# afanasyev-ilya/VectorGraphLibrary

Hardware: AMD Instinct MI355X
Metric: TEPS (edges/s) BFS + SSSP on RMAT-24; value = direction-optimising BFS, sssp_value_teps = direction-optimising Bellman-Ford (higher is better)
Workload: dtype int32; 1 GPU; BFS direction-optimising on RMAT scale-24 (edge factor 32), 1xMI355X; vertices=16777216, edges=536870912, seed=1, parallelism=edge-cut x1, exchange_transport=none, vertex_numbering=degree-sorted (total)

## Files before the change

### profiles/microbench/bfs_launches.py

```python
#!/usr/bin/env python3
import csv
import glob
import sys

files = sorted(glob.glob(sys.argv[1] + "/**/*kernel_trace.csv", recursive=True))
rows = []
for f in files:
    with open(f) as fh:
        for r in csv.DictReader(fh):
            rows.append((int(r["Start_Timestamp"]), int(r["End_Timestamp"]), r["Kernel_Name"].split("(")[0]))
rows.sort()
short = {"vgl_k_bu_probe": "probe", "vgl_k_bu_heavy": "heavy", "vgl_k_bm_advance": "adv", "vgl_k_td_expand": "td"}
inits = [i for i, r in enumerate(rows) if "bfs_init" in r[2]]
n = int(sys.argv[2]) if len(sys.argv) > 2 else 3
spans = [(a, b) for a, b in zip(inits[:-1], inits[1:]) if any("bu_probe" in r[2] for r in rows[a:b])]
for a, b in spans[-n:]:
    t0 = rows[a][0]
    parts, prev_end, busy = [], None, 0
    for s, e, name in rows[a:b]:
        label = next((v for k, v in short.items() if k in name), name.replace('void ', '').replace('vgl_k_', '')[:14])
        gap = "" if prev_end is None else f"(+{(s - prev_end) / 1e3:.1f})"
        parts.append(f"{label} {(e - s) / 1e3:.1f}{gap}")
        busy += e - s
        prev_end = e
    span = rows[b - 1][1] - t0
    print("traversal: " + "  ".join(parts) + f"   | span {span / 1e3:.1f} us, kernels {busy / 1e3:.1f} us, idle {(span - busy) / 1e3:.1f} us")
```

### vectorgraphlibrary_amd/csrc/bfs.hip

```cpp
#include "vgl_hip_internal.h"
#include <chrono>
#include "vgl_gnf.h"
#include "vgl_blocked.h"

#ifndef VGL_BU_HEAVY_LANES
#define VGL_BU_HEAVY_LANES 16
#endif

__global__ __launch_bounds__(VGL_BLOCK) void vgl_k_bfs_init(int32_t V, int32_t source, int32_t *levels)
{
    for (int32_t v = blockIdx.x * VGL_BLOCK + threadIdx.x; v < V; v += gridDim.x * VGL_BLOCK)
        levels[v] = (v == source) ? 1 : -1;
}

__global__ __launch_bounds__(VGL_BLOCK) void vgl_k_bfs_init_all(int32_t V, int32_t source, int32_t *levels, int64_t words, uint64_t *visited,
                                                                uint64_t *front, uint64_t *next, uint32_t *tickets, unsigned long long *list_count)
{
    if (blockIdx.x == 0 && threadIdx.x == 0) *list_count = 0ULL;
    for (int32_t v = blockIdx.x * VGL_BLOCK + threadIdx.x; v < V; v += gridDim.x * VGL_BLOCK)
        levels[v] = (v == source) ? 1 : -1;
    for (int64_t w = (int64_t)blockIdx.x * VGL_BLOCK + threadIdx.x; w < words; w += (int64_t)gridDim.x * VGL_BLOCK) {
        const uint64_t bit = (w == (source >> 6)) ? (1ULL << (source & 63)) : 0ULL;
        visited[w] = bit; front[w] = bit; next[w] = 0;
    }
// ... 556 lines not shown
            for (int u = 0; u < U; u++) {
                const unsigned long long bit = dst[u] >= 0 ? 1ULL << (dst[u] & 63) : 0ULL;
                old[u] = (word[u] & bit) || dst[u] < 0 ? ~0ULL : atomicOr((unsigned long long *)&visited[dst[u] >> 6], bit);
            }
#pragma unroll
            for (int u = 0; u < U; u++) {
                if (dst[u] < 0) continue;
                const unsigned long long bit = 1ULL << (dst[u] & 63);
                if (old[u] & bit) continue;
                levels[dst[u]] = level + 1;
                atomicOr((unsigned long long *)&next[dst[u] >> 6], bit);
                const int pos = atomicAdd(&s_cnt, 1);
                if (pos < VGL_SMALL_F) s_list[cur ^ 1][pos] = dst[u];
                else found_deg += rowptr[dst[u] + 1] - rowptr[dst[u]];
            }
        }
        __syncthreads();
        const int32_t Fn = s_cnt;
        edges += M; run++; last_f = F;
        if (run > 1) later_front += F;
        F = Fn;
        if (Fn > VGL_SMALL_F) {
            {
                static_assert(VGL_SMALL_F == 2 * NT, "two listed vertices per thread");
                const int32_t v0 = s_list[cur ^ 1][tid], v1 = s_list[cur ^ 1][tid + NT];
                const int64_t a0 = rowptr[v0], a1 = rowptr[v0 + 1], c0 = rowptr[v1], c1 = rowptr[v1 + 1];
                found_deg += (a1 - a0) + (c1 - c0);
            }
            found_deg = vgl_wave_incl_add(found_deg);
            if (lane == 63) s_deg[wave] = found_deg;
            __syncthreads();
#pragma unroll
            for (int w = 0; w < NW; w++) next_m += s_deg[w];
            hinted = 1;
            break;
        }
        if (Fn == 0) break;
        cur ^= 1; level++;
    }
    if (tid == 0) {
        counters[C_FRONT] = F; counters[C_TMP0] = run; counters[C_EDGES] = edges; counters[C_TMP1] = later_front; counters[C_JUMP] = last_f;
        counters[C_NEIGH] = first_m; counters[C_BU_FOUND] = n_list; counters[C_CHANGED] = bm_edges;
        if (hinted) { counters[C_NEXT_F] = F; counters[C_NEXT_M] = next_m; }
        host[C_HINT] = hinted;
        host[C_FRONT] = F; host[C_TMP0] = run; host[C_EDGES] = edges; host[C_TMP1] = later_front; host[C_JUMP] = last_f; host[C_NEIGH] = first_m;
        host[C_BU_FOUND] = n_list; host[C_CHANGED] = bm_edges; host[C_HEAVY] = handed; host[C_BU_EDGES] = exit_m;
        __threadfence_system();
        host[C_NSLOTS] = seq;
        __threadfence_system();
    }
}

constexpr int VGL_BU_BLOCKS = 2048;

typedef int vgl_int4_u __attribute__((ext_vector_type(4), aligned(4)));

typedef unsigned vgl_uint3_u __attribute__((ext_vector_type(3), aligned(4)));
template <bool PACKED>
__device__ __forceinline__ void vgl_load_head(const int4 *in_head, int64_t rec, int32_t u[4])
{
    if constexpr (PACKED) {
        const vgl_uint3_u w = *reinterpret_cast<const vgl_uint3_u *>(reinterpret_cast<const uint32_t *>(in_head) + 3 * rec);
        const uint32_t f[4] = {w.x & 0xFFFFFFu, (w.x >> 24) | ((w.y & 0xFFFFu) << 8), (w.y >> 16) | ((w.z & 0xFFu) << 16), w.z >> 8};
#pragma unroll
        for (int q = 0; q < 4; q++) u[q] = f[q] == 0xFFFFFFu ? -1 : (int32_t)f[q];
    } else {
        const int4 h = in_head[rec];
        u[0] = h.x; u[1] = h.y; u[2] = h.z; u[3] = h.w;
    }
}
template <bool INLINE_HEAVY, bool PACKED>
__device__ __forceinline__ void vgl_bu_probe_body(int32_t nrows, int32_t row_base, int32_t chunk, const int64_t *in_rowptr,
                                                  const int32_t *in_adj, const uint64_t *visited, const uint64_t *in_nz,
                                                  const uint64_t *front, uint64_t *next, int32_t *levels, int32_t next_level,
                                                  int32_t *heavy, int64_t *partials, uint32_t *ticket, const int4 *in_head,
                                                  const uint64_t *in_long, const int32_t *nz_rank, int32_t nz_rows, int64_t *counters,
                                                  volatile int64_t *host, int64_t seq)
{
    static_assert(INLINE_HEAVY, "the deferred rows are scanned in the same launch");
    __shared__ int64_t s64[VGL_WAVES];
    __shared__ int s_nheavy;
    if (threadIdx.x == 0) s_nheavy = 0;
    __syncthreads();
    auto in_front = [&](int32_t u) -> uint32_t { return (uint32_t)((front[u >> 6] >> (u & 63)) & 1ULL); };
    int64_t found_cnt = 0, probes = 0;
    const int64_t groups = ((int64_t)nrows + 63) >> 6;
    const int64_t word0 = (int64_t)row_base >> 6;
    constexpr int64_t NW = (int64_t)VGL_BU_BLOCKS * VGL_WAVES;
    int32_t *my_heavy = heavy + (int64_t)blockIdx.x * chunk;
    const int lane = vgl_lane();
    for (int64_t g0 = (int64_t)blockIdx.x * VGL_WAVES + vgl_wave(); g0 < groups; g0 += NW * 64) {
        const int64_t mine = g0 + (int64_t)lane * NW;
        uint64_t cw = 0, nzw = 0;
        int32_t nzr = 0;
        if (mine < groups) {
            nzw = in_nz[word0 + mine];
            cw = ~visited[word0 + mine] & nzw;
            if (cw == 0ULL) next[word0 + mine] = 0ULL;
            else nzr = nz_rank[mine];
        }
        unsigned long long todo = __ballot(cw != 0ULL);
        while (todo) {
            const int j = __ffsll((long long)todo) - 1;
            todo &= todo - 1;
            const uint64_t cand_word = __shfl(cw, j);
            const int32_t rec = __shfl(nzr, j) + (int32_t)__popcll(__shfl(nzw, j) & ((1ULL << lane) - 1ULL));
            const int64_t grp = g0 + (int64_t)j * NW;
            const int32_t r = (int32_t)(grp << 6) + lane;
            const int32_t v = row_base + r;
            bool found = false, defer = false;
            if (r < nrows && ((cand_word >> lane) & 1ULL)) {
                int32_t u0[4];
                vgl_load_head<PACKED>(in_head, rec, u0);
                uint32_t hit = 0;
                int n = 0;
#pragma unroll
                for (int q = 0; q < 4; q++) if (u0[q] >= 0) n = q + 1;
                if (u0[0] >= 0) hit = in_front(u0[0]);
                if (hit == 0) {
#pragma unroll
                    for (int q = 1; q < 4; q++)
                        if (u0[q] >= 0) hit |= in_front(u0[q]) << q;
                }
                bool longer = false;
                if (hit == 0 && n == 4) {
                    int32_t u1[4];
                    vgl_load_head<PACKED>(in_head, (int64_t)nz_rows + rec, u1);
#pragma unroll
                    for (int q = 0; q < 4; q++)
                        if (u1[q] >= 0) { n = 5 + q; hit |= in_front(u1[q]) << (4 + q); }
                    longer = (in_long[v >> 6] >> (v & 63)) & 1ULL;
                }
                found = hit != 0;
                probes += found ? __ffs(hit) : n;
                defer = !found && longer;
                if (found) levels[v] = next_level;
            }
            const unsigned long long fm = __ballot(found);
            if (lane == 0) next[word0 + grp] = fm;
            found_cnt += found;
            const unsigned long long dm = __ballot(defer);
            if (dm) {
                int base = 0;
                if (lane == 0) base = atomicAdd(&s_nheavy, (int)__popcll(dm));
                base = __shfl(base, 0);
                if (defer) my_heavy[base + __popcll(dm & ((1ULL << lane) - 1ULL))] = r;
            }
        }
    }
    __syncthreads();
    const int nh = s_nheavy;
    constexpr int G = VGL_BU_HEAVY_LANES, NG = 64 / G;
    const int quarter = lane / G, ql = lane % G;
    for (int h0 = vgl_wave() * NG; h0 < nh; h0 += VGL_WAVES * NG) {
        const int h = h0 + quarter;
        bool done = h >= nh, hit_any = false;
        int32_t r = 0;
        int64_t p = 0, e = 0;
        if (!done) { r = my_heavy[h]; p = in_rowptr[r]; e = in_rowptr[r + 1]; }
        while (!__all(done)) {
            const int64_t q = p + ql;
            bool hit = false;
            if (!done && q < e) { const int32_t u = in_adj[q]; hit = (front[u >> 6] >> (u & 63)) & 1ULL; }
            const unsigned long long hm = __ballot(hit);
            const unsigned qm = (unsigned)(hm >> (quarter * G)) & (G >= 32 ? 0xFFFFFFFFu : ((1u << (G & 31)) - 1u));
            if (!done) {
                if (qm) { hit_any = true; done = true; if (ql == 0) probes += __ffs(qm); }
                else { if (ql == 0) probes += min((int64_t)G, e - p); p += G; if (p >= e) done = true; }
            }
        }
        if (hit_any && ql == 0) {
            const int32_t v = row_base + r;
            levels[v] = next_level;
            atomicOr((unsigned long long *)&next[v >> 6], 1ULL << (v & 63));
            found_cnt++;
        }
    }
    found_cnt = vgl_block_reduce_add(found_cnt, s64);
    probes = vgl_block_reduce_add(probes, s64);
    uint32_t dep = 0;
    if (threadIdx.x == 0) dep = vgl_put_agent(partials + blockIdx.x * 4 + 0, found_cnt) ^ vgl_put_agent(partials + blockIdx.x * 4 + 1, probes);
    if (!vgl_last_block(ticket, dep)) return;
    int64_t f = 0, pr = 0;
    for (int b = threadIdx.x; b < (int)gridDim.x; b += VGL_BLOCK) { f += vgl_load_agent(partials + b * 4 + 0); pr += vgl_load_agent(partials + b * 4 + 1); }
    f = vgl_block_reduce_add(f, s64);
    pr = vgl_block_reduce_add(pr, s64);
    if (threadIdx.x == 0) {
        if (host) vgl_publish2(counters, host, seq, C_BU_FOUND, f, C_BU_EDGES, pr);
        else { counters[C_BU_FOUND] = f; counters[C_BU_EDGES] = pr; }
    }
}
#define VGL_BU_PROBE_PARAMS                                                                                                                             \
    int32_t nrows, int32_t row_base, int32_t chunk, const int64_t *in_rowptr, const int32_t *in_adj, const uint64_t *visited, const uint64_t *in_nz,  \
        const uint64_t *front, uint64_t *next, int32_t *levels, int32_t next_level, int32_t *heavy, int64_t *partials, uint32_t *ticket,               \
        const int4 *in_head, const uint64_t *in_long, const int32_t *nz_rank, int32_t nz_rows, int64_t *counters, volatile int64_t *host, int64_t seq
#define VGL_BU_PROBE_ARGS                                                                                                                               \
    nrows, row_base, chunk, in_rowptr, in_adj, visited, in_nz, front, next, levels, next_level, heavy, partials, ticket, in_head, in_long, nz_rank,    \
        nz_rows, counters, host, seq
template <bool INLINE_HEAVY>
__global__ __launch_bounds__(VGL_BLOCK) __attribute__((amdgpu_num_sgpr(80))) void vgl_k_bu_probe(VGL_BU_PROBE_PARAMS)
{
    vgl_bu_probe_body<INLINE_HEAVY, true>(VGL_BU_PROBE_ARGS);
}
template <bool INLINE_HEAVY>
__global__ __launch_bounds__(VGL_BLOCK) void vgl_k_bu_probe_wide(VGL_BU_PROBE_PARAMS)
{
    vgl_bu_probe_body<INLINE_HEAVY, false>(VGL_BU_PROBE_ARGS);
}

__global__ __launch_bounds__(VGL_BLOCK) void vgl_k_bm_advance(int64_t words, uint64_t *visited, uint64_t *front, uint64_t *next)
{
    for (int64_t w = (int64_t)blockIdx.x * VGL_BLOCK + threadIdx.x; w < words; w += (int64_t)gridDim.x * VGL_BLOCK) {
        const uint64_t n = next[w];
        if (n) { visited[w] |= n; next[w] = 0; }
        front[w] = n;
    }
}

constexpr int VGL_B2I_BLOCKS = 2048;
__global__ __launch_bounds__(VGL_BLOCK) void vgl_k_bitmap_to_ids(int64_t words, const uint64_t *bits, int64_t word_base, int32_t cap, int32_t *out)
{
    __shared__ int s32[VGL_WAVES];
    __shared__ int s_base;
    const int64_t per = (((words + gridDim.x - 1) / gridDim.x + VGL_BLOCK - 1) / VGL_BLOCK) * VGL_BLOCK;
    const int64_t lo = (int64_t)blockIdx.x * per, hi = min(words, lo + per);
    int n = 0;
    for (int64_t wi = lo + threadIdx.x; wi < hi; wi += VGL_BLOCK) n += (int)__popcll(bits[wi]);
    int total = 0;
    vgl_block_excl_add(n, s32, &total);
    if (total == 0) return;
    if (threadIdx.x == 0) s_base = atomicAdd(out, total);
    __syncthreads();
    int run = s_base;
    for (int64_t w0 = lo; w0 < hi && run < cap; w0 += VGL_BLOCK) {
        const int64_t wi = w0 + threadIdx.x;
        uint64_t w = wi < hi ? bits[wi] : 0ULL;
        int step = 0;
        int pos = run + vgl_block_excl_add((int)__popcll(w), s32, &step);
        while (w) {
            const int b = __ffsll((long long)w) - 1;
            w &= w - 1;
            if (pos < cap) out[1 + pos] = (int32_t)(((word_base + wi) << 6) + b);
            pos++;
        }
        run += step;
    }
}
__global__ __launch_bounds__(VGL_BLOCK) void vgl_k_apply_ids(int32_t V, int parts, int32_t cap, const int32_t *lists, int32_t *levels, int32_t level,
                                                             uint64_t *visited, uint64_t *front, const int32_t *degrees, int64_t *partials)
{
    __shared__ int64_t s64[VGL_WAVES];
    int64_t cnt = 0, deg = 0;
    const int64_t total = (int64_t)parts * cap;
    for (int64_t t = (int64_t)blockIdx.x * VGL_BLOCK + threadIdx.x; t < total; t += (int64_t)gridDim.x * VGL_BLOCK) {
        const int p = (int)(t / cap), i = (int)(t % cap);
        const int32_t *list = lists + (int64_t)p * (1 + cap);
        if (i >= list[0]) continue;
        const int32_t v = list[1 + i];
        if (v < 0 || v >= V) continue;
        const unsigned long long bit = 1ULL << (v & 63);
// ... 98 lines not shown
                       COUNT ? g->tickets + 3 * VGL_TICKET_WORDS : (uint32_t *)nullptr, COUNT ? c->d_counters : (int64_t *)nullptr);
}

constexpr int64_t VGL_TD_COUNT_TILES = 8192;
static int vgl_bfs_td_launch(vgl_hip_ctx *c, vgl_hip_graph *g, int32_t F, int64_t M, int32_t *levels, int32_t next_level, bool emit,
                             bool have_tile_first, bool count = false, bool filter = true)
{
    if (F <= 0 || M <= 0) return 0;
    if (!have_tile_first) hipLaunchKernelGGL(vgl_k_tile_first, dim3(vgl_grid(F, VGL_BLOCK, 8192)), dim3(VGL_BLOCK), 0, c->stream, F, g->offs, g->tile_first);
    {
        vgl_timed_launch tl(c, "bfs_top_down");
        if (emit && count) vgl_td_expand_launch<true, true>(c, g, F, M, g->bm_visited, levels, next_level, g->bm_next, filter);
        else if (emit) vgl_td_expand_launch<true, false>(c, g, F, M, g->bm_visited, levels, next_level, g->bm_next, filter);
        else vgl_td_expand_launch<false, false>(c, g, F, M, g->bm_visited, levels, next_level, g->bm_next, filter);
    }
    VGL_HIP_TRY(hipGetLastError());
    return 0;
}

int vgl_bfs_bm_gnf(vgl_hip_ctx *c, vgl_hip_graph *g, const uint64_t *front, bool count, bool write, int64_t M_known, bool advance, const vgl_do_hint *hint)
{
    const vgl_do_hint no_hint = {0, 0, 0, 0};
    const int64_t word0 = g->row_begin >> 6;
    const int64_t nwords = vgl_ceil_div(g->row_end, 64) - word0;
    const unsigned nb = (unsigned)vgl_ceil_div(nwords, VGL_BLOCK);
    if (count) {
        const int64_t seq = vgl_next_seq(c);
        {
            vgl_timed_launch tl(c, "gnf");
            if (advance)
                hipLaunchKernelGGL(vgl_k_bm_gnf_count<true>, dim3(nb), dim3(VGL_BLOCK), 0, c->stream, nwords, word0, g->row_begin, g->bm_front,
                                   g->out.rowptr, g->vt_cnt, g->vt_deg, g->vt_cnt_off, g->vt_deg_off, g->offs, c->d_counters,
                                   g->tickets + 0 * VGL_TICKET_WORDS, (volatile int64_t *)c->h_counters, seq, g->bm_visited, g->bm_next,
                                   hint ? 1 : 0, hint ? *hint : no_hint);
            else
                hipLaunchKernelGGL(vgl_k_bm_gnf_count<false>, dim3(nb), dim3(VGL_BLOCK), 0, c->stream, nwords, word0, g->row_begin,
                                   const_cast<uint64_t *>(front), g->out.rowptr, g->vt_cnt, g->vt_deg, g->vt_cnt_off, g->vt_deg_off, g->offs, c->d_counters,
                                   g->tickets + 0 * VGL_TICKET_WORDS, (volatile int64_t *)c->h_counters, seq, (uint64_t *)nullptr, (uint64_t *)nullptr,
                                   0, no_hint);
        }
        VGL_HIP_TRY(hipGetLastError());
        VGL_TRY(vgl_wait_counters(c, seq));
    }
    if (write) {
        vgl_timed_launch tl(c, "gnf");
        hipLaunchKernelGGL(vgl_k_bm_gnf_write, dim3(nb), dim3(VGL_BLOCK), 0, c->stream, nwords, word0, g->row_begin, front,
                           g->out.rowptr, g->vt_cnt_off, g->vt_deg_off, g->ids, g->offs, g->tile_first, M_known >= 0 ? M_known : c->h_counters[C_NEIGH]);
        VGL_HIP_TRY(hipGetLastError());
    }
    return 0;
}

static int vgl_bfs_bu_launch(vgl_hip_ctx *c, vgl_hip_graph *g, int32_t *levels, int32_t next_level, const uint64_t *visited,
                             const uint64_t *front, uint64_t *next, int64_t *seq_out)
{
    const int32_t chunk = (int32_t)(vgl_ceil_div(vgl_ceil_div(g->nrows, VGL_BU_BLOCKS), VGL_BLOCK) * VGL_BLOCK);
    const int64_t seq = vgl_next_seq(c);
    {
        vgl_timed_launch tl(c, "bfs_bottom_up");
        auto *kernel = g->in_head_packed ? vgl_k_bu_probe<true> : vgl_k_bu_probe_wide<true>;
        hipLaunchKernelGGL(kernel, dim3(VGL_BU_BLOCKS), dim3(VGL_BLOCK), 0, c->stream, g->nrows, g->row_begin, chunk,
                           g->in.rowptr, g->in.adj, visited, g->bm_in_nz, front, next, levels, next_level, g->heavy, g->bu_partials,
                           g->tickets + 1 * VGL_TICKET_WORDS, reinterpret_cast<const int4 *>(g->in_head.p), g->bm_in_long,
                           (const int32_t *)g->in_nz_rank, g->in_nz_rows, c->d_counters, (volatile int64_t *)c->h_counters, seq);
    }
    VGL_HIP_TRY(hipGetLastError());
    if (seq_out) *seq_out = seq;
    return 0;
}

static int vgl_bfs_blocked_level(vgl_hip_ctx *c, vgl_hip_graph *g, int32_t *levels, int32_t next_level)
{
    for (const vgl_blocked_piece &p : g->blk_bfs->pieces) {
        if (p.n_g_units > 0) {
            vgl_timed_launch tl(c, "bfs_blk_gather");
            hipLaunchKernelGGL(vgl_k_bfs_blk_gather, dim3((unsigned)p.n_g_units), dim3(VGL_BTHREADS), 0, c->stream, (const vgl_blk_unit *)p.g_units,
                               (const uint16_t *)p.g_lo, (const uint32_t *)p.mid_to_a, reinterpret_cast<uint64_t *>(p.vals.p), p.g_count,
                               (const uint64_t *)g->bm_front, (int64_t)g->row_begin >> 6);
        }
        if (p.n_a_units > 0) {
            vgl_timed_launch tl(c, "bfs_blk_accumulate");
            hipLaunchKernelGGL(vgl_k_bfs_blk_accumulate, dim3((unsigned)p.n_a_units), dim3(VGL_BTHREADS), 0, c->stream, (const vgl_blk_unit *)p.a_units,
                               (const uint16_t *)p.a_lo, reinterpret_cast<const uint64_t *>(p.vals.p), p.a_count, (const uint64_t *)g->bm_visited,
                               g->bm_next, levels, next_level);
        }
    }
    VGL_HIP_TRY(hipGetLastError());
    return 0;
}

__global__ __launch_bounds__(VGL_BLOCK) void vgl_k_zero_words(int64_t words, uint64_t *p)
{
    for (int64_t i = (int64_t)blockIdx.x * VGL_BLOCK + threadIdx.x; i < words; i += (int64_t)gridDim.x * VGL_BLOCK) p[i] = 0ULL;
}
int vgl_zero_words(vgl_hip_ctx *c, uint64_t *d_words, int64_t words)
{
    if (words > 0)
        hipLaunchKernelGGL(vgl_k_zero_words, dim3((unsigned)std::min<int64_t>(4096, vgl_ceil_div(words, VGL_BLOCK))), dim3(VGL_BLOCK), 0, c->stream, words, d_words);
    VGL_HIP_TRY(hipGetLastError());
    return 0;
}

int vgl_bitmap_to_ids(vgl_hip_ctx *c, int64_t words, const uint64_t *d_bits, int64_t word_base, int32_t cap, int32_t *d_out)
{
    VGL_HIP_TRY(hipMemsetAsync(d_out, 0, sizeof(int32_t), c->stream));
    if (words > 0) {
        vgl_timed_launch tl(c, "bfs_shard_resolve");
        hipLaunchKernelGGL(vgl_k_bitmap_to_ids, dim3((unsigned)std::min<int64_t>(VGL_B2I_BLOCKS, vgl_ceil_div(words, VGL_BLOCK))), dim3(VGL_BLOCK), 0, c->stream,
                           words, d_bits, word_base, cap, d_out);
    }
    VGL_HIP_TRY(hipGetLastError());
    return 0;
}

static int64_t vgl_bfs_td_emit_edges(int64_t V) { return std::max<int64_t>(65536, V / 256); }

struct vgl_bfs_params {
    int64_t td_emit_edges;
    double td_filter_share;
    double td_late_share;
    double blocked_share;
    int64_t small_m;
    int64_t bm_expand_f;
    bool use_hints, scan_bound, trace;
};
static vgl_bfs_params vgl_bfs_params_of(const vgl_bfs_tunables &tn, int64_t V, int mode)
{
    const bool do_mode = mode == VGL_HIP_BFS_DIRECTION_OPT;
    vgl_bfs_params p;
    p.td_emit_edges = tn.td_emit_edges >= 0 ? tn.td_emit_edges : vgl_bfs_td_emit_edges(V);
    p.td_filter_share = tn.td_filter_share >= 0.0 ? tn.td_filter_share : 0.125;
    p.td_late_share = tn.td_late_share >= 0.0 ? tn.td_late_share : 1.0 / 64;
    p.blocked_share = tn.blocked_share >= 0.0 ? tn.blocked_share : 0.1;
    p.small_m = tn.small_m >= 0 ? std::min<int64_t>(tn.small_m, 1 << 20) : 8192;
    if (do_mode) p.small_m = std::min<int64_t>(p.small_m, vgl_do_bottom_up_edges(V, V, 1) - 1);
    if (p.small_m < 64) p.small_m = 0;
    p.bm_expand_f = tn.bm_expand >= 0 ? tn.bm_expand : 262144;
    if (vgl_ceil_div(vgl_ceil_div(V, 64), VGL_BLOCK) > 8192) p.bm_expand_f = 0;
    p.use_hints = do_mode && !tn.no_hint;
    p.scan_bound = do_mode && !tn.no_scan_bound;
    p.trace = tn.trace;
    return p;
}

enum class vgl_bfs_front {
    levels,
    pending,
    bitmap,
    counted_bitmap,
    counted_scan,
    ids,
};

struct vgl_bfs_traversal {
    vgl_hip_ctx *c;
    vgl_hip_graph *g;
    int mode;
    int32_t *levels;
    vgl_bfs_params p;
    int32_t V;
    int64_t E, words, factor;
    unsigned bm_blocks;
    unsigned long long *list_count;
    std::chrono::steady_clock::time_point t0;

    int32_t cur = 1;
    vgl_bfs_front front = vgl_bfs_front::bitmap;
    bool bottom_up = false;
    bool hint_ready = false, skipped = false, finished = false;
    int64_t F = 0, M = 0, prevF = 0, visited_total = 0;
    vgl_hip_bfs_stats st = {0, 0, 0, 0, 0, 0, 0, 0, 0, 0, 0};

    vgl_bfs_traversal(vgl_hip_ctx *c_, vgl_hip_graph *g_, int mode_, int32_t *levels_)
        : c(c_), g(g_), mode(mode_), levels(levels_), p(vgl_bfs_params_of(c_->bfs, g_->V, mode_)), V(g_->V), E(g_->out.edges)
    {
        words = vgl_ceil_div(V, 64);
        factor = vgl_do_factor(E, V);
        bm_blocks = (unsigned)vgl_ceil_div(words, VGL_BLOCK);
        list_count = reinterpret_cast<unsigned long long *>(c->d_counters + C_HEAVY);
    }

    void trace(const char *what)
    {
        if (!p.trace) return;
        hipStreamSynchronize(c->stream);
        fprintf(stderr, "[bfs trace] %7.3f ms  level %d  F %lld  M %lld  visited %lld  %s\n",
                std::chrono::duration<double, std::milli>(std::chrono::steady_clock::now() - t0).count(), (int)cur, (long long)F, (long long)M,
                (long long)visited_total, what);
    }
    void begin_level(int64_t f) { visited_total += f; st.levels++; st.frontier_total += f; }
    void book_top_down(int64_t f, int64_t m) { st.td_steps++; st.edges_examined += m; st.td_edges += m; st.td_frontier += f; }
    bool late() const
    {
        if (g->in_nz_rows <= 0 || p.td_late_share <= 0.0) return false;
        const int64_t remain = std::max<int64_t>(0, (int64_t)g->in_nz_rows + 1 - visited_total);
        return (double)remain <= p.td_late_share * (double)V;
    }

    int count()
    {
        trace("-> count");
        skipped = false;
        const char *done = "count done (bitmap)";
        if (front != vgl_bfs_front::levels) {
            const bool advance = front == vgl_bfs_front::pending;
            const vgl_do_hint hint = {prevF, visited_total, (int64_t)V, factor};
            const bool hinted = hint_ready && advance && p.use_hints;
            VGL_TRY(vgl_bfs_bm_gnf(c, g, g->bm_front, true, false, -1, advance, hinted ? &hint : nullptr));
            skipped = hinted && c->h_counters[C_SKIPPED] != 0;
            front = skipped ? vgl_bfs_front::bitmap : vgl_bfs_front::counted_bitmap;
        } else if (p.scan_bound && g->nvtiles <= 8192) {
            const int64_t seq = vgl_next_seq(c);
            {
                vgl_timed_launch tl(c, "gnf");
                hipLaunchKernelGGL(vgl_k_bfs_scan_bound, dim3((unsigned)g->nvtiles), dim3(VGL_BLOCK), 0, c->stream, g->nrows, g->row_begin, (const int32_t *)levels,
                                   cur, (const int32_t *)g->vt_min_deg, (uint8_t *)g->bm_front.p, (uint8_t *)g->bm_visited.p, g->bu_partials,
                                   g->tickets + 0 * VGL_TICKET_WORDS, c->d_counters, (volatile int64_t *)c->h_counters, seq);
            }
            VGL_HIP_TRY(hipGetLastError());
            VGL_TRY(vgl_wait_counters(c, seq));
            front = vgl_bfs_front::bitmap;
            const int64_t f = c->h_counters[C_FRONT], m_lb = c->h_counters[C_NEIGH];
            if (vgl_do_turn_bottom_up(f, m_lb, prevF, visited_total + f, V, factor)) {
                F = f; M = m_lb; skipped = true; hint_ready = false;
                trace("count done (levels scan)");
                return 0;
            }
            VGL_TRY(vgl_bfs_bm_gnf(c, g, g->bm_front, true, false, -1, false, nullptr));
            front = vgl_bfs_front::counted_bitmap;
        } else {
            vgl_pred_equal_i32 pred{levels, cur};
            VGL_TRY(vgl_gnf_run(c, g, pred, g->ids, g->offs, (uint8_t *)g->bm_front.p, (uint8_t *)g->bm_visited.p, nullptr, false, true));
            front = vgl_bfs_front::counted_scan;
            done = "count done (levels scan)";
        }
        F = c->h_counters[C_FRONT]; M = c->h_counters[C_NEIGH];
        hint_ready = false;
        trace(done);
        return 0;
    }

    int small_levels(int32_t listF, int32_t src, bool from_bitmap)
    {
        if (from_bitmap) {
            vgl_timed_launch tl(c, "bfs_bitmap_expand");
            hipLaunchKernelGGL(vgl_k_bm_expand, dim3(bm_blocks), dim3(VGL_BLOCK), 0, c->stream, words, g->bm_front, g->out.rowptr, g->out.adj, g->bm_visited,
                               g->bm_next, levels, cur + 1, g->ids, list_count, (int32_t)VGL_SMALL_F, g->bu_partials);
        }
        const int64_t seq = vgl_next_seq(c);
// ... 38 lines not shown
        } else front = vgl_bfs_front::pending;
        return 0;
    }
    int blocked_level()
    {
        trace("counted -> blocked level");
        VGL_TRY(vgl_bfs_blocked_level(c, g, levels, cur + 1));
        trace("blocked level done");
        front = vgl_bfs_front::pending;
        book_top_down(F, M);
        cur++;
        return 0;
    }
    int top_down_level()
    {
        switch (front) {
        case vgl_bfs_front::ids: break;
        case vgl_bfs_front::counted_bitmap: VGL_TRY(vgl_bfs_bm_gnf(c, g, g->bm_front, false, true, M)); break;
        case vgl_bfs_front::counted_scan: {
            vgl_pred_equal_i32 pred{levels, cur};
            vgl_timed_launch tl(c, "gnf");
            hipLaunchKernelGGL(vgl_k_gnf_write<vgl_pred_equal_i32>, dim3((unsigned)g->nvtiles), dim3(VGL_BLOCK), 0, c->stream, pred,
                               g->nrows, g->row_begin, g->out.rowptr, g->vt_cnt_off, g->vt_deg_off, g->ids, g->offs, (int32_t *)nullptr, (int64_t)0);
            break;
        }
        default: VGL_FAIL("bfs_run: internal error (frontier not counted)");
        }
        trace("ids written");
        const bool have_tile_first = front != vgl_bfs_front::counted_scan;
        if (p.small_m > 0 && have_tile_first && F <= VGL_SMALL_F && M <= p.small_m) {
            trace("counted + ids -> list kernel");
            VGL_TRY(small_levels((int32_t)F, -1, false));
            trace("list kernel done");
            book_small(F);
            return 0;
        }
        const bool is_late = late();
        const bool emit = M <= p.td_emit_edges || is_late;
        const bool td_counts = emit && p.use_hints && vgl_ceil_div(M, VGL_TILE) <= VGL_TD_COUNT_TILES;
        const bool filter = is_late || (double)visited_total >= p.td_filter_share * (double)V;
        trace(emit ? "counted + ids -> top-down (emitting)" : "counted + ids -> top-down (levels only)");
        VGL_TRY(vgl_bfs_td_launch(c, g, (int32_t)F, M, levels, cur + 1, emit, have_tile_first, td_counts, filter));
        trace("top-down done");
        hint_ready = td_counts && F > 0 && M > 0;
        front = emit ? vgl_bfs_front::pending : vgl_bfs_front::levels;
        book_top_down(F, M);
        cur++;
        return 0;
    }
    int bottom_up_level()
    {
        if (front == vgl_bfs_front::levels || front == vgl_bfs_front::pending) VGL_FAIL("bfs_run: internal error (bitmaps missing)");
        int64_t seq = 0;
        trace("-> bottom-up");
        VGL_TRY(vgl_bfs_bu_launch(c, g, levels, cur + 1, g->bm_visited, g->bm_front, g->bm_next, &seq));
        hipLaunchKernelGGL(vgl_k_bm_advance, dim3(vgl_grid(words, VGL_BLOCK, 8192)), dim3(VGL_BLOCK), 0, c->stream, words, g->bm_visited, g->bm_front, g->bm_next);
        VGL_HIP_TRY(hipGetLastError());
        VGL_TRY(vgl_wait_counters(c, seq));
        st.bu_steps++; st.edges_examined += c->h_counters[C_BU_EDGES];
        st.bu_edges += c->h_counters[C_BU_EDGES]; st.bu_found += c->h_counters[C_BU_FOUND];
        F = c->h_counters[C_BU_FOUND]; M = 0;
        front = vgl_bfs_front::bitmap;
        cur++;
        return 0;
    }

    int run(int32_t source)
    {
        hipLaunchKernelGGL(vgl_k_bfs_init_all, dim3(vgl_grid(V, VGL_BLOCK, 8192)), dim3(VGL_BLOCK), 0, c->stream, V, source, levels, words, g->bm_visited, g->bm_front,
                           g->bm_next, g->tickets, list_count);
        t0 = std::chrono::steady_clock::now();
        if (p.small_m > 0) {
            VGL_TRY(small_levels(1, source, false));
            if (c->h_counters[C_TMP0] > 0) {
                begin_level(1);
                prevF = 1;
                book_small(1);
            }
        }
        while (!finished) {
            if (front != vgl_bfs_front::ids && !bottom_up) VGL_TRY(count());
            if (F == 0) break;
            begin_level(F);
            if (mode == VGL_HIP_BFS_DIRECTION_OPT) {
                if (!bottom_up) bottom_up = vgl_do_turn_bottom_up(F, M, prevF, visited_total, V, factor);
                else if (vgl_do_turn_top_down(F, prevF, visited_total, V, factor)) {
                    bottom_up = false;
                    if (p.small_m > 0 && F <= p.bm_expand_f) {
                        VGL_TRY(expand_from_bitmap());
                        continue;
                    }
                    VGL_TRY(count());
                }
            }
            if (!bottom_up && front == vgl_bfs_front::counted_bitmap && p.small_m > 0 && F <= p.bm_expand_f && late()) {
                VGL_TRY(expand_from_bitmap());
                continue;
            }
            prevF = F;
            if (skipped && !bottom_up) VGL_FAIL("bfs_run: internal error (the count launch and the host disagree on the direction rule)");
            if (bottom_up) VGL_TRY(bottom_up_level());
            else if (g->blk_bfs && front != vgl_bfs_front::levels && (double)M >= p.blocked_share * (double)E) VGL_TRY(blocked_level());
            else VGL_TRY(top_down_level());
        }
        st.discovered = visited_total;
        st.algorithmic_bytes = 8 * st.edges_examined + 20 * st.frontier_total + 4 * st.discovered + 4 * (int64_t)V +
                               (int64_t)st.bu_steps * (V / 8);
        return 0;
// ... 200 lines not shown
```

### vectorgraphlibrary_amd/csrc/context.hip

```cpp
#include "vgl_hip_internal.h"
#include <unordered_set>
#include <cstdio>
#include <cstring>
#include <mutex>
#include <algorithm>

static thread_local std::string g_last_error;

int vgl_set_error(const char *file, int line, const char *msg)
{
    char buf[512];
    const char *base = strrchr(file, '/');
    snprintf(buf, sizeof(buf), "vgl_hip: %s (%s:%d)", msg, base ? base + 1 : file, line);
    g_last_error = buf;
    return 1;
}

static hipMemPool_t g_lib_pool[64];
static bool g_lib_pool_tried[64];
static std::mutex g_lib_pool_mutex;
hipMemPool_t vgl_lib_pool(int device)
{
    if (device < 0 || device >= 64) return nullptr;
    std::lock_guard<std::mutex> lock(g_lib_pool_mutex);
// ... 3 lines not shown
        memset(&props, 0, sizeof(props));
        props.allocType = hipMemAllocationTypePinned;
        props.handleTypes = hipMemHandleTypeNone;
        props.location.type = hipMemLocationTypeDevice;
        props.location.id = device;
        hipMemPool_t pool = nullptr;
        if (hipMemPoolCreate(&pool, &props) == hipSuccess && pool) {
            uint64_t keep = 48ULL << 30;
            if (const char *e = getenv("VGL_POOL_KEEP_GB")) keep = (uint64_t)std::max(0.0, atof(e)) << 30;
            (void)hipMemPoolSetAttribute(pool, hipMemPoolAttrReleaseThreshold, &keep);
            g_lib_pool[device] = pool;
        } else (void)hipGetLastError();
    }
    return g_lib_pool[device];
}

static std::mutex g_big_mutex;
static std::unordered_set<void *> g_big_blocks;
size_t vgl_pool_block_limit()
{
    static const size_t limit = [] { const char *e = getenv("VGL_POOL_MAX_MB"); return (e ? (size_t)strtoull(e, nullptr, 10) : (size_t)64) << 20; }();
    return limit;
}
void vgl_big_block_remember(void *p) { std::lock_guard<std::mutex> lock(g_big_mutex); g_big_blocks.insert(p); }
bool vgl_big_block_forget(void *p) { std::lock_guard<std::mutex> lock(g_big_mutex); return g_big_blocks.erase(p) != 0; }

extern char **environ;
static uint64_t vgl_env_signature()
{
    uint64_t h = 1469598103934665603ull ^ (uint64_t)(uintptr_t)environ;
    if (environ) for (char **e = environ; *e; e++) h = (h ^ (uint64_t)(uintptr_t)*e) * 1099511628211ull;
    return h ? h : 1;
}
void vgl_ctx_refresh_env(vgl_hip_ctx *c)
{
    const uint64_t sig = vgl_env_signature();
    if (sig == c->env_signature) return;
    c->env_signature = sig;
    c->env.clear();
    if (environ)
        for (char **e = environ; *e; e++)
            if (strncmp(*e, "VGL_", 4) == 0)
                if (const char *eq = strchr(*e, '=')) c->env[std::string(*e, (size_t)(eq - *e))] = std::string(eq + 1);
    vgl_bfs_tunables t;
    auto str = [&](const char *n) -> const char * { auto it = c->env.find(n); return it == c->env.end() ? nullptr : it->second.c_str(); };
    auto on = [&](const char *n) { const char *v = str(n); return v && v[0] == '1'; };
    if (const char *v = str("VGL_TD_EMIT_EDGES")) t.td_emit_edges = atoll(v);
    if (const char *v = str("VGL_BFS_SMALL_M")) t.small_m = atoll(v);
    if (const char *v = str("VGL_BFS_BM_EXPAND")) t.bm_expand = atoll(v);
    if (const char *v = str("VGL_SHARD_TD_EMIT_EDGES")) t.shard_td_emit_edges = atoll(v);
    if (const char *v = str("VGL_TD_FILTER_SHARE")) t.td_filter_share = atof(v);
    if (const char *v = str("VGL_TD_LATE_SHARE")) t.td_late_share = atof(v);
    if (const char *v = str("VGL_BFS_BLOCKED_SHARE")) t.blocked_share = atof(v);
    if (const char *v = str("VGL_SHARD_SPARSE_CAP")) t.shard_sparse_cap = std::max(0, atoi(v));
    t.no_hint = on("VGL_BFS_NO_HINT"); t.no_scan_bound = on("VGL_BFS_NO_SCAN_BOUND"); t.trace = on("VGL_BFS_TRACE");
    c->bfs = t;
}
const char *vgl_env(vgl_hip_ctx *c, const char *name)
{
    vgl_ctx_refresh_env(c);
    auto it = c->env.find(name);
    return it == c->env.end() ? nullptr : it->second.c_str();
}
int64_t vgl_env_int(vgl_hip_ctx *c, const char *name, int64_t dflt, int64_t lo, int64_t hi)
{
    const char *s = vgl_env(c, name);
    const int64_t v = (s && *s) ? strtoll(s, nullptr, 10) : dflt;
    return std::min(hi, std::max(lo, v));
}

extern "C" {

int vgl_hip_abi_version(void) { return VGL_HIP_ABI_VERSION; }
const char *vgl_hip_last_error(void) { return g_last_error.c_str(); }

int vgl_hip_ctx_create(int device, void *stream, vgl_hip_ctx **out)
{
    if (!out) VGL_FAIL("ctx_create: null out pointer");
    int ndev = 0;
    VGL_HIP_TRY(hipGetDeviceCount(&ndev));
    if (ndev <= 0) VGL_FAIL("no HIP device visible: the MI355X backend has no CPU fallback");
    if (device < 0 || device >= ndev) VGL_FAIL("ctx_create: device index out of range");
    VGL_HIP_TRY(hipSetDevice(device));
    vgl_hip_ctx *c = new vgl_hip_ctx();
    c->device = device;
    c->stream = (hipStream_t)stream;
    c->own_stream = false;
    VGL_HIP_TRY(hipMalloc((void **)&c->d_counters, sizeof(int64_t) * C_NSLOTS));
    VGL_HIP_TRY(hipHostMalloc((void **)&c->h_counters, sizeof(int64_t) * (C_NSLOTS + 8), hipHostMallocDefault));
    VGL_HIP_TRY(hipMemsetAsync(c->d_counters, 0, sizeof(int64_t) * C_NSLOTS, c->stream));
    VGL_HIP_TRY(hipMalloc((void **)&c->d_shards, sizeof(int64_t) * VGL_NSHARD));
    VGL_HIP_TRY(hipMemsetAsync(c->d_shards, 0, sizeof(int64_t) * VGL_NSHARD, c->stream));
    memset(c->h_counters, 0, sizeof(int64_t) * (C_NSLOTS + 8));
    vgl_ctx_refresh_env(c);
    *out = c;
    return 0;
}

int vgl_hip_ctx_trim(vgl_hip_ctx *c)
{
    if (!c) VGL_FAIL("null context");
    VGL_HIP_TRY(hipStreamSynchronize(c->stream));
    if (hipMemPool_t pool = vgl_lib_pool(c->device)) VGL_HIP_TRY(hipMemPoolTrimTo(pool, 0));
    return 0;
}

// ... 207 lines not shown
```

### vectorgraphlibrary_amd/csrc/vgl_hip_internal.h

```cpp
#pragma once
#include <hip/hip_runtime.h>
#include <stdint.h>
#include <string>
#include <map>
#include <memory>
#include <vector>
#include "../../include/vgl_hip.h"

constexpr int VGL_BLOCK = 256;
constexpr int VGL_EPT = 8;
constexpr int VGL_TILE = VGL_BLOCK * VGL_EPT;
constexpr int VGL_WAVES = VGL_BLOCK / 64;

int vgl_set_error(const char *file, int line, const char *msg);
#define VGL_FAIL(msg) return vgl_set_error(__FILE__, __LINE__, (msg))
#define VGL_HIP_TRY(expr)                                                          \
    do {                                                                           \
        hipError_t _e = (expr);                                                    \
        if (_e != hipSuccess) return vgl_set_error(__FILE__, __LINE__, hipGetErrorString(_e)); \
    } while (0)
#define VGL_TRY(expr)            \
    do {                         \
        int _s = (expr);         \
        if (_s != 0) return _s;  \
    } while (0)

enum {
    C_FRONT = 0, C_NEIGH = 1, C_BU_FOUND = 2, C_BU_EDGES = 3, C_HEAVY = 4, C_CHANGED = 5,
    C_EDGES = 6, C_TMP0 = 7, C_TMP1 = 8, C_JUMP = 9,
    C_NEXT_F = 10, C_NEXT_M = 11,
    C_SKIPPED = 12, C_HINT = 13,
    C_NSLOTS = 32
};
constexpr int VGL_NSHARD = 1024;

struct vgl_timing_slot {
    int64_t launches = 0;
    std::vector<std::pair<hipEvent_t, hipEvent_t>> pending;
    double total_ms = 0.0;
};

struct vgl_bfs_tunables {
    int64_t td_emit_edges = -1, small_m = -1, bm_expand = -1, shard_td_emit_edges = -1;
    double td_filter_share = -1.0, td_late_share = -1.0, blocked_share = -1.0;
    int shard_sparse_cap = -1;
    bool no_hint = false, no_scan_bound = false, trace = false;
};

struct vgl_hip_ctx {
    std::map<std::string, std::string> env;
    uint64_t env_signature = 0;
    vgl_bfs_tunables bfs;
    int device = 0;
    hipStream_t stream = nullptr;
    bool own_stream = false;
    int64_t *d_counters = nullptr;
    int64_t *d_shards = nullptr;
    int64_t *h_counters = nullptr;
    int64_t publish_seq = 0;
    double *d_partials = nullptr;
    size_t partials_cap = 0;
    bool timing = false;
    std::string timing_only;
    int timing_stride = 1;
    int64_t timing_seen = 0;
    std::map<std::string, vgl_timing_slot> slots;
    std::vector<hipEvent_t> event_pool;
};

void vgl_ctx_refresh_env(vgl_hip_ctx *c);
const char *vgl_env(vgl_hip_ctx *c, const char *name);
int64_t vgl_env_int(vgl_hip_ctx *c, const char *name, int64_t dflt, int64_t lo, int64_t hi);

hipMemPool_t vgl_lib_pool(int device);
size_t vgl_pool_block_limit();
void vgl_big_block_remember(void *p);
bool vgl_big_block_forget(void *p);
static inline hipError_t vgl_pool_alloc(hipStream_t st, void **p, size_t bytes)
{
    if (bytes >= vgl_pool_block_limit()) {
        const hipError_t e = hipMalloc(p, bytes);
        if (e == hipSuccess) vgl_big_block_remember(*p);
        return e;
    }
    int dev = 0;
    if (hipGetDevice(&dev) == hipSuccess)
        if (hipMemPool_t pool = vgl_lib_pool(dev)) return hipMallocFromPoolAsync(p, bytes ? bytes : 16, pool, st);
    return hipMallocAsync(p, bytes ? bytes : 16, st);
}
static inline void vgl_pool_free(hipStream_t st, void *p)
{
    if (!p) return;
    if (vgl_big_block_forget(p)) { (void)hipStreamSynchronize(st); (void)hipFree(p); }
    else (void)hipFreeAsync(p, st);
}
template <class T>
struct vgl_dev {
// ... 349 lines not shown
```

Baseline: 1788 billion edges/s.

## Add compacted sparse bottom-up probe kernel for late BFS levels

```diff
diff --git a/profiles/microbench/bfs_launches.py b/profiles/microbench/bfs_launches.py
--- a/profiles/microbench/bfs_launches.py
+++ b/profiles/microbench/bfs_launches.py
@@ -10,7 +10,7 @@
         for r in csv.DictReader(fh):
             rows.append((int(r["Start_Timestamp"]), int(r["End_Timestamp"]), r["Kernel_Name"].split("(")[0]))
 rows.sort()
-short = {"vgl_k_bu_probe": "probe", "vgl_k_bu_heavy": "heavy", "vgl_k_bm_advance": "adv", "vgl_k_td_expand": "td"}
+short = {"vgl_k_bu_probe_sparse": "sprobe", "vgl_k_bu_probe": "probe", "vgl_k_bu_heavy": "heavy", "vgl_k_bm_advance": "adv", "vgl_k_td_expand": "td"}
 inits = [i for i, r in enumerate(rows) if "bfs_init" in r[2]]
 n = int(sys.argv[2]) if len(sys.argv) > 2 else 3
 spans = [(a, b) for a, b in zip(inits[:-1], inits[1:]) if any("bu_probe" in r[2] for r in rows[a:b])]
diff --git a/vectorgraphlibrary_amd/csrc/bfs.hip b/vectorgraphlibrary_amd/csrc/bfs.hip
--- a/vectorgraphlibrary_amd/csrc/bfs.hip
+++ b/vectorgraphlibrary_amd/csrc/bfs.hip
@@ -632,6 +632,7 @@
 }
 
 constexpr int VGL_BU_BLOCKS = 2048;
+constexpr double VGL_BU_SPARSE_SHARE_DEFAULT = 0.25;
 
 typedef int vgl_int4_u __attribute__((ext_vector_type(4), aligned(4)));
 
@@ -649,7 +650,60 @@
         u[0] = h.x; u[1] = h.y; u[2] = h.z; u[3] = h.w;
     }
 }
-template <bool INLINE_HEAVY, bool PACKED>
+template <bool PACKED>
+__device__ __forceinline__ void vgl_bu_probe_row(const int4 *in_head, const uint64_t *front, const uint64_t *in_long, int32_t nz_rows, int32_t rec,
+                                                 int32_t v, int32_t *levels, int32_t next_level, int64_t &probes, bool &found, bool &defer)
+{
+    auto in_front = [&](int32_t u) -> uint32_t { return (uint32_t)((front[u >> 6] >> (u & 63)) & 1ULL); };
+    int32_t u0[4];
+    vgl_load_head<PACKED>(in_head, rec, u0);
+    uint32_t hit = 0;
+    int n = 0;
+#pragma unroll
+    for (int q = 0; q < 4; q++) if (u0[q] >= 0) n = q + 1;
+    if (u0[0] >= 0) hit = in_front(u0[0]);
+    if (hit == 0) {
+#pragma unroll
+        for (int q = 1; q < 4; q++)
+            if (u0[q] >= 0) hit |= in_front(u0[q]) << q;
+    }
+    bool longer = false;
+    if (hit == 0 && n == 4) {
+        int32_t u1[4];
+        vgl_load_head<PACKED>(in_head, (int64_t)nz_rows + rec, u1);
+#pragma unroll
+        for (int q = 0; q < 4; q++)
+            if (u1[q] >= 0) { n = 5 + q; hit |= in_front(u1[q]) << (4 + q); }
+        longer = (in_long[v >> 6] >> (v & 63)) & 1ULL;
+    }
+    found = hit != 0;
+    probes += found ? __ffs(hit) : n;
+    defer = !found && longer;
+    if (found) levels[v] = next_level;
+}
+__device__ __forceinline__ void vgl_bu_defer_rows(bool defer, int32_t r, int lane, int *s_nheavy, int32_t *my_heavy)
+{
+    const unsigned long long dm = __ballot(defer);
+    if (dm) {
+        int base = 0;
+        if (lane == 0) base = atomicAdd(s_nheavy, (int)__popcll(dm));
+        base = __shfl(base, 0);
+        if (defer) my_heavy[base + __popcll(dm & ((1ULL << lane) - 1ULL))] = r;
+    }
+}
+__device__ __forceinline__ int vgl_select_bit64(uint64_t w, int n)
+{
+    uint32_t x = (uint32_t)w;
+    int pos = 0, c = __popc(x);
+    if (n >= c) { n -= c; pos = 32; x = (uint32_t)(w >> 32); }
+#pragma unroll
+    for (int h = 16; h >= 1; h >>= 1) {
+        c = __popc(x & ((1u << h) - 1u));
+        if (n >= c) { n -= c; pos += h; x >>= h; }
+    }
+    return pos;
+}
+template <bool INLINE_HEAVY, bool PACKED, bool SPARSE>
 __device__ __forceinline__ void vgl_bu_probe_body(int32_t nrows, int32_t row_base, int32_t chunk, const int64_t *in_rowptr,
                                                   const int32_t *in_adj, const uint64_t *visited, const uint64_t *in_nz,
                                                   const uint64_t *front, uint64_t *next, int32_t *levels, int32_t next_level,
@@ -662,7 +716,6 @@
     __shared__ int s_nheavy;
     if (threadIdx.x == 0) s_nheavy = 0;
     __syncthreads();
-    auto in_front = [&](int32_t u) -> uint32_t { return (uint32_t)((front[u >> 6] >> (u & 63)) & 1ULL); };
     int64_t found_cnt = 0, probes = 0;
     const int64_t groups = ((int64_t)nrows + 63) >> 6;
     const int64_t word0 = (int64_t)row_base >> 6;
@@ -676,8 +729,45 @@
         if (mine < groups) {
             nzw = in_nz[word0 + mine];
             cw = ~visited[word0 + mine] & nzw;
-            if (cw == 0ULL) next[word0 + mine] = 0ULL;
+            if (cw == 0ULL) { if constexpr (!SPARSE) next[word0 + mine] = 0ULL; }
             else nzr = nz_rank[mine];
+        }
+        if constexpr (SPARSE) {
+            __shared__ unsigned long long s_fm[VGL_WAVES][64];
+            unsigned long long *my_fm = s_fm[vgl_wave()];
+            if (mine == groups - 1 && (nrows & 63)) cw &= (1ULL << (nrows & 63)) - 1ULL;
+            my_fm[lane] = 0ULL;
+            __builtin_amdgcn_fence(__ATOMIC_ACQ_REL, "wavefront");
+            __builtin_amdgcn_wave_barrier();
+            const int incl = vgl_wave_incl_add((int)__popcll(cw));
+            const int T = __shfl(incl, 63);
+            for (int b = 0; b < T; b += 64) {
+                const bool active = b + lane < T;
+                const int k = active ? b + lane : T - 1;
+                int j = 0;
+#pragma unroll
+                for (int h = 32; h >= 1; h >>= 1) {
+                    const int at = __shfl(incl, j + h - 1);
+                    j += at <= k ? h : 0;
+                }
+                const uint64_t cand_word = __shfl(cw, j), nz_word = __shfl(nzw, j);
+                const int bit = vgl_select_bit64(cand_word, k - (__shfl(incl, j) - (int)__popcll(cand_word)));
+                const int32_t rec = __shfl(nzr, j) + (int32_t)__popcll(nz_word & ((1ULL << bit) - 1ULL));
+                const int64_t grp = g0 + (int64_t)j * NW;
+                const int32_t r = (int32_t)(grp << 6) + bit;
+                const int32_t v = row_base + r;
+                bool found = false, defer = false;
+                if (active && r < nrows) {
+                    vgl_bu_probe_row<PACKED>(in_head, front, in_long, nz_rows, rec, v, levels, next_level, probes, found, defer);
+                }
+                if (found) atomicOr(&my_fm[j], 1ULL << bit);
+                found_cnt += found;
+                vgl_bu_defer_rows(defer, r, lane, &s_nheavy, my_heavy);
+            }
+            __builtin_amdgcn_fence(__ATOMIC_ACQ_REL, "wavefront");
+            __builtin_amdgcn_wave_barrier();
+            if (mine < groups) next[word0 + mine] = my_fm[lane];
+            continue;
         }
         unsigned long long todo = __ballot(cw != 0ULL);
         while (todo) {
@@ -690,42 +780,12 @@
             const int32_t v = row_base + r;
             bool found = false, defer = false;
             if (r < nrows && ((cand_word >> lane) & 1ULL)) {
-                int32_t u0[4];
-                vgl_load_head<PACKED>(in_head, rec, u0);
-                uint32_t hit = 0;
-                int n = 0;
-#pragma unroll
-                for (int q = 0; q < 4; q++) if (u0[q] >= 0) n = q + 1;
-                if (u0[0] >= 0) hit = in_front(u0[0]);
-                if (hit == 0) {
-#pragma unroll
-                    for (int q = 1; q < 4; q++)
-                        if (u0[q] >= 0) hit |= in_front(u0[q]) << q;
-                }
-                bool longer = false;
-                if (hit == 0 && n == 4) {
-                    int32_t u1[4];
-                    vgl_load_head<PACKED>(in_head, (int64_t)nz_rows + rec, u1);
-#pragma unroll
-                    for (int q = 0; q < 4; q++)
-                        if (u1[q] >= 0) { n = 5 + q; hit |= in_front(u1[q]) << (4 + q); }
-                    longer = (in_long[v >> 6] >> (v & 63)) & 1ULL;
-                }
-                found = hit != 0;
-                probes += found ? __ffs(hit) : n;
-                defer = !found && longer;
-                if (found) levels[v] = next_level;
+                vgl_bu_probe_row<PACKED>(in_head, front, in_long, nz_rows, rec, v, levels, next_level, probes, found, defer);
             }
             const unsigned long long fm = __ballot(found);
             if (lane == 0) next[word0 + grp] = fm;
             found_cnt += found;
-            const unsigned long long dm = __ballot(defer);
-            if (dm) {
-                int base = 0;
-                if (lane == 0) base = atomicAdd(&s_nheavy, (int)__popcll(dm));
-                base = __shfl(base, 0);
-                if (defer) my_heavy[base + __popcll(dm & ((1ULL << lane) - 1ULL))] = r;
-            }
+            vgl_bu_defer_rows(defer, r, lane, &s_nheavy, my_heavy);
         }
     }
     __syncthreads();
@@ -780,12 +840,22 @@
 template <bool INLINE_HEAVY>
 __global__ __launch_bounds__(VGL_BLOCK) __attribute__((amdgpu_num_sgpr(80))) void vgl_k_bu_probe(VGL_BU_PROBE_PARAMS)
 {
-    vgl_bu_probe_body<INLINE_HEAVY, true>(VGL_BU_PROBE_ARGS);
+    vgl_bu_probe_body<INLINE_HEAVY, true, false>(VGL_BU_PROBE_ARGS);
 }
 template <bool INLINE_HEAVY>
 __global__ __launch_bounds__(VGL_BLOCK) void vgl_k_bu_probe_wide(VGL_BU_PROBE_PARAMS)
 {
-    vgl_bu_probe_body<INLINE_HEAVY, false>(VGL_BU_PROBE_ARGS);
+    vgl_bu_probe_body<INLINE_HEAVY, false, false>(VGL_BU_PROBE_ARGS);
+}
+template <bool INLINE_HEAVY>
+__global__ __launch_bounds__(VGL_BLOCK) __attribute__((amdgpu_num_sgpr(80))) void vgl_k_bu_probe_sparse(VGL_BU_PROBE_PARAMS)
+{
+    vgl_bu_probe_body<INLINE_HEAVY, true, true>(VGL_BU_PROBE_ARGS);
+}
+template <bool INLINE_HEAVY>
+__global__ __launch_bounds__(VGL_BLOCK) __attribute__((amdgpu_num_sgpr(80))) void vgl_k_bu_probe_sparse_wide(VGL_BU_PROBE_PARAMS)
+{
+    vgl_bu_probe_body<INLINE_HEAVY, false, true>(VGL_BU_PROBE_ARGS);
 }
 
 __global__ __launch_bounds__(VGL_BLOCK) void vgl_k_bm_advance(int64_t words, uint64_t *visited, uint64_t *front, uint64_t *next)
@@ -990,13 +1060,14 @@
 }
 
 static int vgl_bfs_bu_launch(vgl_hip_ctx *c, vgl_hip_graph *g, int32_t *levels, int32_t next_level, const uint64_t *visited,
-                             const uint64_t *front, uint64_t *next, int64_t *seq_out)
+                             const uint64_t *front, uint64_t *next, int64_t *seq_out, bool sparse = false)
 {
     const int32_t chunk = (int32_t)(vgl_ceil_div(vgl_ceil_div(g->nrows, VGL_BU_BLOCKS), VGL_BLOCK) * VGL_BLOCK);
     const int64_t seq = vgl_next_seq(c);
     {
         vgl_timed_launch tl(c, "bfs_bottom_up");
-        auto *kernel = g->in_head_packed ? vgl_k_bu_probe<true> : vgl_k_bu_probe_wide<true>;
+        auto *kernel = g->in_head_packed ? (sparse ? vgl_k_bu_probe_sparse<true> : vgl_k_bu_probe<true>)
+                                         : (sparse ? vgl_k_bu_probe_sparse_wide<true> : vgl_k_bu_probe_wide<true>);
         hipLaunchKernelGGL(kernel, dim3(VGL_BU_BLOCKS), dim3(VGL_BLOCK), 0, c->stream, g->nrows, g->row_begin, chunk,
                            g->in.rowptr, g->in.adj, visited, g->bm_in_nz, front, next, levels, next_level, g->heavy, g->bu_partials,
                            g->tickets + 1 * VGL_TICKET_WORDS, reinterpret_cast<const int4 *>(g->in_head.p), g->bm_in_long,
@@ -1058,6 +1129,7 @@
     double td_filter_share;
     double td_late_share;
     double blocked_share;
+    double bu_sparse_share;
     int64_t small_m;
     int64_t bm_expand_f;
     bool use_hints, scan_bound, trace;
@@ -1070,6 +1142,7 @@
     p.td_filter_share = tn.td_filter_share >= 0.0 ? tn.td_filter_share : 0.125;
     p.td_late_share = tn.td_late_share >= 0.0 ? tn.td_late_share : 1.0 / 64;
     p.blocked_share = tn.blocked_share >= 0.0 ? tn.blocked_share : 0.1;
+    p.bu_sparse_share = tn.bu_sparse_share >= 0.0 ? tn.bu_sparse_share : VGL_BU_SPARSE_SHARE_DEFAULT;
     p.small_m = tn.small_m >= 0 ? std::min<int64_t>(tn.small_m, 1 << 20) : 8192;
     if (do_mode) p.small_m = std::min<int64_t>(p.small_m, vgl_do_bottom_up_edges(V, V, 1) - 1);
     if (p.small_m < 64) p.small_m = 0;
@@ -1128,11 +1201,16 @@
     }
     void begin_level(int64_t f) { visited_total += f; st.levels++; st.frontier_total += f; }
     void book_top_down(int64_t f, int64_t m) { st.td_steps++; st.edges_examined += m; st.td_edges += m; st.td_frontier += f; }
+    int64_t remain() const { return std::max<int64_t>(0, (int64_t)g->in_nz_rows + 1 - visited_total); }
     bool late() const
     {
         if (g->in_nz_rows <= 0 || p.td_late_share <= 0.0) return false;
-        const int64_t remain = std::max<int64_t>(0, (int64_t)g->in_nz_rows + 1 - visited_total);
-        return (double)remain <= p.td_late_share * (double)V;
+        return (double)remain() <= p.td_late_share * (double)V;
+    }
+    bool sparse_bottom_up() const
+    {
+        if (p.bu_sparse_share <= 0.0) return false;
+        return p.bu_sparse_share >= 1.0 || (double)remain() <= p.bu_sparse_share * (double)g->in_nz_rows;
     }
 
     int count()
@@ -1277,8 +1355,9 @@
     {
         if (front == vgl_bfs_front::levels || front == vgl_bfs_front::pending) VGL_FAIL("bfs_run: internal error (bitmaps missing)");
         int64_t seq = 0;
-        trace("-> bottom-up");
-        VGL_TRY(vgl_bfs_bu_launch(c, g, levels, cur + 1, g->bm_visited, g->bm_front, g->bm_next, &seq));
+        const bool sparse = sparse_bottom_up();
+        trace(sparse ? "-> bottom-up (sparse probe)" : "-> bottom-up");
+        VGL_TRY(vgl_bfs_bu_launch(c, g, levels, cur + 1, g->bm_visited, g->bm_front, g->bm_next, &seq, sparse));
         hipLaunchKernelGGL(vgl_k_bm_advance, dim3(vgl_grid(words, VGL_BLOCK, 8192)), dim3(VGL_BLOCK), 0, c->stream, words, g->bm_visited, g->bm_front, g->bm_next);
         VGL_HIP_TRY(hipGetLastError());
         VGL_TRY(vgl_wait_counters(c, seq));
diff --git a/vectorgraphlibrary_amd/csrc/context.hip b/vectorgraphlibrary_amd/csrc/context.hip
--- a/vectorgraphlibrary_amd/csrc/context.hip
+++ b/vectorgraphlibrary_amd/csrc/context.hip
@@ -79,6 +79,7 @@
     if (const char *v = str("VGL_TD_FILTER_SHARE")) t.td_filter_share = atof(v);
     if (const char *v = str("VGL_TD_LATE_SHARE")) t.td_late_share = atof(v);
     if (const char *v = str("VGL_BFS_BLOCKED_SHARE")) t.blocked_share = atof(v);
+    if (const char *v = str("VGL_BFS_BU_SPARSE_SHARE")) t.bu_sparse_share = atof(v);
     if (const char *v = str("VGL_SHARD_SPARSE_CAP")) t.shard_sparse_cap = std::max(0, atoi(v));
     t.no_hint = on("VGL_BFS_NO_HINT"); t.no_scan_bound = on("VGL_BFS_NO_SCAN_BOUND"); t.trace = on("VGL_BFS_TRACE");
     c->bfs = t;
diff --git a/vectorgraphlibrary_amd/csrc/vgl_hip_internal.h b/vectorgraphlibrary_amd/csrc/vgl_hip_internal.h
--- a/vectorgraphlibrary_amd/csrc/vgl_hip_internal.h
+++ b/vectorgraphlibrary_amd/csrc/vgl_hip_internal.h
@@ -42,7 +42,7 @@
 
 struct vgl_bfs_tunables {
     int64_t td_emit_edges = -1, small_m = -1, bm_expand = -1, shard_td_emit_edges = -1;
-    double td_filter_share = -1.0, td_late_share = -1.0, blocked_share = -1.0;
+    double td_filter_share = -1.0, td_late_share = -1.0, blocked_share = -1.0, bu_sparse_share = -1.0;
     int shard_sparse_cap = -1;
     bool no_hint = false, no_scan_bound = false, trace = false;
 };
```

After: 1824 billion edges/s, median of 4. 2.0% higher.
